# steineggerlab/Metabuli

Hardware: AMD Instinct MI355X
Metric: Mreads/s classified (metabuli classify hot path, reads + index resident in HBM) (higher is better)
Workload: dtype u64

## Files before the change

### metabuli_amd/csrc/kernels_score.h

```cpp
#ifndef MTB_KERNELS_SCORE_H
#define MTB_KERNELS_SCORE_H
#include "dev_util.h"
#include "mtb_core.h"
#include "kernels_join.h"
#include "mtb_score_par.h"

#ifdef MTB_SCORE_PHASE_CYCLES
#define MTB_NPHASE 16
__device__ unsigned long long mtb_phase_cycles[MTB_NPHASE];
__shared__ unsigned long long mtb_phase_lds[MTB_NPHASE];
#define MTB_PHASE_BEGIN() unsigned long long ph_t0_ = __builtin_readcyclecounter()
#define MTB_PHASE_MARK(k) do { unsigned long long t_ = __builtin_readcyclecounter(); if (threadIdx.x == 0) mtb_phase_lds[k] += t_ - ph_t0_; ph_t0_ = t_; } while (0)
#define MTB_PHASE_KERNEL_BEGIN() do { if (threadIdx.x < MTB_NPHASE) mtb_phase_lds[threadIdx.x] = 0; __syncthreads(); } while (0)
#define MTB_PHASE_KERNEL_END() do { __syncthreads(); if (threadIdx.x < MTB_NPHASE) atomicAdd(&mtb_phase_cycles[threadIdx.x], mtb_phase_lds[threadIdx.x]); } while (0)
#else
#define MTB_PHASE_BEGIN() do {} while (0)
#define MTB_PHASE_MARK(k) do {} while (0)
#define MTB_PHASE_KERNEL_BEGIN() do {} while (0)
#define MTB_PHASE_KERNEL_END() do {} while (0)
#endif

#ifndef MTB_SCORE_LDS
#define MTB_SCORE_LDS 160
#endif
// ... 6 lines not shown
    uint64_t b = mtb_sws_bytes<uint32_t>(n);
    b += nb * 12 + (MTB_LR_MAXE + MTB_LR_MAXE * MTB_LR_K) * 4 + ((nb + 15) & ~15ull);
    return (b + 63) & ~63ull;
}

__global__ __launch_bounds__(64) void k_taxcnt_bound(const uint64_t *__restrict__ seg_start, const uint32_t *__restrict__ cursor,
                                                      const int32_t *__restrict__ qlen, const int32_t *__restrict__ qlen2, uint64_t n_reads,
                                                      int32_t dna_shift, uint32_t *__restrict__ bound) {
    uint64_t r = (uint64_t)blockIdx.x * 64 + threadIdx.x;
    if (r >= n_reads) return;
    uint64_t nb = (uint64_t)mtb_num_buckets(qlen[r] + qlen2[r], dna_shift);
    if (cursor) { bound[r] = (uint32_t)nb; return; }
    uint64_t n = seg_start[r + 1] - seg_start[r];
    bound[r] = (uint32_t)(n < nb ? n : nb);
}

__global__ __launch_bounds__(256) void k_count_flags(const uint8_t *__restrict__ f, uint64_t n, unsigned long long *__restrict__ out) {
    uint32_t c = 0;
    for (uint64_t i = (uint64_t)blockIdx.x * 256 + threadIdx.x; i < n; i += (uint64_t)gridDim.x * 256) c += f[i] == 1 ? 1u : 0u;
    for (int d = 32; d > 0; d >>= 1) c += __shfl_down(c, d, 64);
    if ((threadIdx.x & 63) == 0 && c) atomicAdd(out, (unsigned long long)c);
}

__global__ __launch_bounds__(256) void k_list_flag2(const uint8_t *__restrict__ f, uint64_t n, uint32_t *__restrict__ list, uint32_t *__restrict__ n_list) {
    __shared__ uint32_t s_w[4]; __shared__ uint32_t s_base;
    const uint64_t r = (uint64_t)blockIdx.x * 256 + threadIdx.x;
    const bool on = r < n && f[r] == 2;
    const uint64_t m = __ballot(on);
    const uint32_t wv = threadIdx.x >> 6, lane = threadIdx.x & 63u;
    if (lane == 0) s_w[wv] = (uint32_t)__popcll(m);
    __syncthreads();
    if (threadIdx.x == 0) { const uint32_t tot = s_w[0] + s_w[1] + s_w[2] + s_w[3]; s_base = tot ? atomicAdd(n_list, tot) : 0u; }
    __syncthreads();
    if (on) {
        uint32_t at = s_base + (uint32_t)__popcll(m & ((1ull << lane) - 1ull));
        for (uint32_t q = 0; q < wv; q++) at += s_w[q];
        list[at] = (uint32_t)r;
    }
}

__global__ __launch_bounds__(256) void k_list_large(const uint64_t *__restrict__ seg_start, uint64_t n_reads, uint32_t threshold,
                                                     uint32_t *__restrict__ large, uint32_t *__restrict__ n_large, uint32_t *__restrict__ max_seg) {
    uint64_t r = (uint64_t)blockIdx.x * 256 + threadIdx.x;
    uint32_t n = 0;
    if (r < n_reads) {
        n = (uint32_t)(seg_start[r + 1] - seg_start[r]);
        if (n > threshold) large[atomicAdd(n_large, 1u)] = (uint32_t)r;
    }
    for (int d = 32; d > 0; d >>= 1) { uint32_t o = __shfl_down(n, d, 64); n = o > n ? o : n; }
    if ((threadIdx.x & 63) == 0 && n > threshold) atomicMax(max_seg, n);
}

__device__ __forceinline__ int32_t taxcnt_gather_wave(const int32_t *btax, const uint8_t *bham, int32_t nb, int32_t *otax, uint32_t *ocnt, int32_t cap) {
    const int32_t lane = (int32_t)threadIdx.x;
    int32_t ntc = 0;
    int32_t last = -1;
    while (ntc < cap) {
        int32_t mn = INT32_MAX;
        for (int32_t q = lane; q < nb; q += 64) if (bham[q] != 255) { int32_t t = btax[q]; if (t > last && t < mn) mn = t; }
        for (int d = 32; d > 0; d >>= 1) { int32_t o = __shfl_xor(mn, d, 64); mn = o < mn ? o : mn; }
// ... 490 lines not shown
                                               mtb_tax_view tx, mtb_score_params sp, const uint64_t *__restrict__ tc_off,
                                               mtb_result *__restrict__ results, int32_t *__restrict__ tc_tax,
                                               uint32_t *__restrict__ tc_cnt, uint64_t tc_cap, uint8_t *__restrict__ slabs,
                                               uint64_t slab_bytes, uint32_t slab_max_n, uint32_t slab_max_nb,
                                               mtb_match *__restrict__ sorted_out, uint64_t tc_base,
                                               const uint32_t *__restrict__ list, const uint32_t *__restrict__ n_list,
                                               const uint32_t *__restrict__ cursor, uint32_t stride, int seg_by_list,
                                               uint32_t direct, uint32_t epoch, uint32_t *__restrict__ big_list, uint32_t *__restrict__ n_big_out,
                                               uint32_t *__restrict__ cnt_out, unsigned long long *__restrict__ work,
                                               const uint8_t *__restrict__ only_flagged, const uint32_t *__restrict__ seg_cnt = nullptr) {
    __shared__ __attribute__((aligned(16))) uint8_t s_ws[MTB_SCORE_WS_BYTES_(CAP)];
    __shared__ uint32_t s_pf[64];
    static_assert(CAP * sizeof(mtb_path) >= MTB_SCORE_BKT * 13 + (MTB_LR_MAXE + MTB_LR_MAXE * MTB_LR_K) * 4, "decide arrays must fit the path area");
    const uint32_t lane = threadIdx.x;
    MTB_BEGIN_ACQUIRE();
    MTB_PHASE_KERNEL_BEGIN();
    const uint64_t n_iter = list ? (uint64_t)*n_list : n_reads;
    for (uint64_t it = DYN ? (uint64_t)__shfl(lane == 0 ? atomicAdd(work, 1ull) : 0ull, 0, 64) : (uint64_t)blockIdx.x; it < n_iter;
         it = DYN ? (uint64_t)__shfl(lane == 0 ? atomicAdd(work, 1ull) : 0ull, 0, 64) : it + gridDim.x) {
#ifdef MTB_SCORE_PHASE_CYCLES
        unsigned long long kt0_ = __builtin_readcyclecounter();
#endif
        const uint64_t r = list ? (uint64_t)list[it] : it;
        if ((SLOT || DYN) && only_flagged && only_flagged[r] != 1) continue;
        if (SLOT && !DYN && !list && !only_flagged && it + gridDim.x < n_iter) {
            const uint32_t lines = (stride * (uint32_t)sizeof(mtb_slot16) + 127u) / 128u;
            if (lane < lines) {
                const uint8_t *pf = (const uint8_t *)((const mtb_slot16 *)matches + (it + gridDim.x) * (uint64_t)stride) + (uint64_t)lane * 128u;
                __builtin_amdgcn_global_load_lds((const __attribute__((address_space(1))) void *)pf,
                                                 (__attribute__((address_space(3))) void *)s_pf, 4, 0, 0);
            }
        }
        uint64_t s0 = 0; int32_t n = 0;
        if (!SLOT) {
            const uint64_t si = seg_by_list ? it : r;
            s0 = seg_start[si]; n = (DYN && seg_cnt) ? (int32_t)seg_cnt[si] : (int32_t)(seg_start[si + 1] - s0);
        }
        const int32_t ql1 = qlen[r], ql2 = qlen2[r];
        const int32_t read_len = ql1 + ql2;
        mtb_result R = mtb_result_blank(ql1, ql2, 0);
        const int32_t nb = mtb_num_buckets(read_len, sp.dna_shift);
        const uint64_t off = tc_off[r], room = tc_off[r + 1] - off;
        if (SLOT) {
            const uint32_t cur = cursor[r], tail_cap = stride - direct;
            mtb_sws<uint16_t> w;
            mtb_sws_carve<uint16_t>(&w, s_ws, CAP);
            bool defer = cur > tail_cap || nb > MTB_SCORE_BKT;
            if (!defer) {
                uint32_t cnt = 0;
                score_sync<uint16_t>();
#ifdef MTB_SCORE_PHASE_CYCLES
// ... 165 lines not shown
```

### metabuli_amd/csrc/kernels_score_fast.h

```cpp
#ifndef MTB_KERNELS_SCORE_FAST_H
#define MTB_KERNELS_SCORE_FAST_H
#include "dev_util.h"
#include "kernels_score.h"
#include "mtb_core.h"
#include "mtb_score_par.h"

#define MTB_FAST_BKT 128
#ifndef MTB_FAST_MERGE_SINGLES
#define MTB_FAST_MERGE_SINGLES 0
#endif

#ifdef MTB_FAST_DEBUG
__device__ unsigned long long mtb_fast_reasons[32];
#define MTB_FAST_COUNT(k, v) do { if (threadIdx.x == 0) atomicAdd(&mtb_fast_reasons[k], (unsigned long long)(v)); } while (0)
#define MTB_FAST_T0() unsigned long long ft_ = __builtin_readcyclecounter()
#define MTB_FAST_MARK(k) do { const unsigned long long t_ = __builtin_readcyclecounter(); if (threadIdx.x == 0) s_ph[k] += t_ - ft_; ft_ = t_; } while (0)
#else
#define MTB_FAST_COUNT(k, v) do {} while (0)
#define MTB_FAST_T0() do {} while (0)
#define MTB_FAST_MARK(k) do {} while (0)
#endif

#define MTB_DPP_RED(v, OP) do { \
    { const uint32_t o_ = (uint32_t)__builtin_amdgcn_update_dpp((int)(v), (int)(v), 0x111, 0xF, 0xF, false); (v) = OP((v), o_); } \
// ... 28 lines not shown
    __shared__ uint64_t s_aux[NMAX];
    __shared__ uint64_t s_pp[NMAX];
    __shared__ FastPath s_path[64];
    __shared__ uint32_t s_pf[64];
    __shared__ uint32_t s_tl[(BYFRAME || MTB_FAST_MERGE_SINGLES) ? 64 : 1];
    typedef uint32_t __attribute__((may_alias)) u32a; typedef int32_t __attribute__((may_alias)) i32a;
    static_assert(NMAX * 8 >= 2 * MTB_FAST_BKT * 4 && NMAX * 8 >= 256 * 4 && NMAX * 8 >= (MTB_LR_MAXE + MTB_LR_MAXE * MTB_LR_K) * 4, "tables fit the arrays they live in");
    u32a *const s_hcnt = (u32a *)s_pp;
    u32a *const s_hmin = (u32a *)s_key; i32a *const s_btax = (i32a *)s_key + MTB_FAST_BKT;
    i32a *const s_otax = (i32a *)s_pp; u32a *const s_ocnt = (u32a *)s_pp + MTB_FAST_BKT;
    i32a *const s_lev = (i32a *)s_aux; i32a *const s_anc = (i32a *)s_aux + MTB_LR_MAXE;
    const int32_t lane = (int32_t)threadIdx.x;
    MTB_BEGIN_ACQUIRE();
#ifdef MTB_FAST_DEBUG
    __shared__ unsigned long long s_ph[16];
    if (threadIdx.x < 16) s_ph[threadIdx.x] = 0;
#endif
    const uint64_t lt = lanemask_lt();
    const uint64_t le = lt | (1ull << lane);
    const uint32_t tail_cap = stride - direct;
    const uint32_t div_m = (65536u + (uint32_t)sp.dna_shift - 1u) / (uint32_t)sp.dna_shift;
    const uint32_t lines = (stride * (uint32_t)sizeof(mtb_slot16) + 127u) / 128u;

    for (uint64_t r = blockIdx.x; r < n_reads; r += gridDim.x) {
        if (r + gridDim.x < n_reads && (uint32_t)lane < lines) {
            const uint8_t *pf = (const uint8_t *)(slots_all + (r + gridDim.x) * (uint64_t)stride) + (uint64_t)lane * 128u;
            __builtin_amdgcn_global_load_lds((const __attribute__((address_space(1))) void *)pf, (__attribute__((address_space(3))) void *)s_pf, 4, 0, 0);
        }
        MTB_FAST_T0();
        const int32_t ql1 = qlen[r], ql2 = qlen2[r];
        const int32_t read_len = ql1 + ql2;
        const int32_t nb = mtb_num_buckets(read_len, sp.dna_shift);
        const uint32_t cur = cursor[r];
        const mtb_slot16 *slots = slots_all + r * (uint64_t)stride;
        mtb_slot16 x[KL];
#pragma unroll
        for (int k = 0; k < KL; k++) { const uint32_t i = (uint32_t)lane + 64u * k; x[k].a = 0; x[k].b = 0; if (i < stride) x[k] = slots[i]; }
        bool slow = cur > tail_cap || nb > MTB_FAST_BKT;
        wave_fence();
        MTB_FAST_MARK(0);
        int32_t n = 0, n_live = 0;
        uint32_t spc[KL]; bool live[KL]; int32_t dst[KL];
        uint32_t smin = 0xFFFFFFFFu, smax = 0u;
#pragma unroll
        for (int k = 0; k < KL; k++) {
            const uint32_t i = (uint32_t)lane + 64u * k;
            live[k] = i < stride && mtb_slot_epoch(x[k]) == epoch && (i < direct || i - direct < cur);
            spc[k] = live[k] ? (uint32_t)(x[k].a >> 32) : 0xFFFFFFFFu;
            dst[k] = 0;
            n_live += (int32_t)__popcll(__ballot(live[k]));
            smin = spc[k] < smin ? spc[k] : smin;
            if (live[k]) smax = spc[k] > smax ? spc[k] : smax;
        }
        smin = wave_min_u32(smin); smax = wave_max_u32(smax);
        uint32_t todo_min = 0xFFFFFFFFu;
        if (smin != smax) {
            for (int32_t q = lane; q < 256; q += 64) s_hcnt[q] = 0;
            wave_fence();
#pragma unroll
            for (int k = 0; k < KL; k++) if (live[k]) atomicAdd(&s_hcnt[(spc[k] * 0x9E3779B1u) >> 24], 1u);
            wave_fence();
// ... 84 lines not shown
                            if (!same_run(ku, kt)) continue;
                            n_tl_less += (less(ku, kt) || (!less(kt, ku) && u < t)) ? 1u : 0u; n_tl_before += u < t ? 1u : 0u;
                        }
                        const int32_t run_start = ti - (int32_t)n_dir_run - (int32_t)n_tl_before;
#pragma unroll
                        for (int k = 0; k < K; k++) if (lane + 64 * k == ti) np[k] = run_start + (int32_t)(n_dir_less + n_tl_less);
                    }
                    wave_fence();
#pragma unroll
                    for (int k = 0; k < K; k++) { const int32_t i = lane + 64 * k; if (k < nsl && i < n) { s_key[np[k]] = ke[k]; s_aux[np[k]] = ax[k] & ~(1ull << 63); } }
                    wave_fence();
                }
            }
        }
        FKey key[K]; uint32_t tid[K], reh[K];
        int32_t tcanon[K]; uint8_t euk[K];
        const mtb_tax_node *nodes = (const mtb_tax_node *)tx.node;
        bool bhead[K], linked[K];
        int32_t shv[K];
        uint64_t bmask[K + 1], lmask[K + 1], rmask[K];
        const int32_t nslot = (n + 63) >> 6;
        bool bad = false, bad2 = false;
#ifdef MTB_FAST_DEBUG
        if (slow) MTB_FAST_COUNT(cur > tail_cap || nb > MTB_FAST_BKT ? 0 : 1, 1);
#endif
#pragma unroll
        for (int k = 0; k < K; k++) {
            const int32_t i = lane + 64 * k;
            key[k].lo = 0; key[k].hi = 0; tid[k] = 0; reh[k] = 0; bhead[k] = true; linked[k] = false; shv[k] = 0; tcanon[k] = -1; euk[k] = 0;
            bmask[k] = ~0ull; lmask[k] = 0; rmask[k] = 0;
            if (k < nslot && !slow) {
                FKey pk; pk.lo = 0; pk.hi = 0;
                if (i < n) {
                    key[k] = s_key[i]; const uint64_t a = s_aux[i]; tid[k] = (uint32_t)a; reh[k] = (uint32_t)(a >> 32) & 0xFFFFu; if (i > 0) pk = s_key[i - 1];
                }
                {
                    const int32_t t_ = (int32_t)tid[k], s_ = (int32_t)fk_species(key[k]);
                    const bool tv = i < n && t_ >= 0 && t_ <= tx.max_taxid, sv = i < n && s_ >= 0 && s_ <= tx.max_taxid;
                    const int32_t tc_ = nodes[tv ? t_ : 0].canon; const uint8_t eu_ = tx.under_euk[sv ? s_ : 0];
                    tcanon[k] = tv ? tc_ : -1; euk[k] = sv ? eu_ : 0;
                }
                const bool first = i == 0;
                if (i < n && !first) {
                    if (pk.hi > key[k].hi || (pk.hi == key[k].hi && pk.lo > key[k].lo)) bad = true;
                    if (pk.hi == key[k].hi && ((pk.lo ^ key[k].lo) >> 27) == 0) bad2 = true;
                }
                bhead[k] = i >= n || first || ((pk.hi ^ key[k].hi) >> 7) != 0;
                if (i < n && !bhead[k]) {
                    const int32_t pos = (int32_t)fk_pos(key[k]), ppos = (int32_t)fk_pos(pk);
                    const int32_t s = (pos - ppos) / 3;
                    if (s > 0 && s <= sp.max_codon_shift) {
                        shv[k] = s;
                        const bool fwd = fk_frame(key[k]) < 3u;
                        linked[k] = mtb_consecutive(fk_dna(pk), fk_dna(key[k]), s, fwd, sp.kmer_format);
                    }
                }
                bmask[k] = __ballot(bhead[k]);
                lmask[k] = __ballot(linked[k]);
                rmask[k] = __ballot(i < n && !linked[k]);
            }
        }
        bmask[K] = ~0ull; lmask[K] = 0;
#ifdef MTB_FAST_DEBUG
        if (!slow) { if (__any(bad)) MTB_FAST_COUNT(2, 1); else if (__any(bad2)) MTB_FAST_COUNT(3, 1); }
#endif
        slow = slow || __any(bad || bad2);
        if (slow) { if (lane == 0) slow_flag[r] = cur > tail_cap ? 2 : 1; continue; }
        if (lane == 0) cnt_out[r] = (uint32_t)n_live;
        MTB_FAST_MARK(2);
        float ps[K]; int32_t phd[K]; int32_t root[K];
        bool cand[K];
        {
            float carry_s = 0.0f; int32_t carry_hd = 0, last_root = 0;
#pragma unroll
            for (int k = 0; k < K; k++) {
                ps[k] = 0.0f; phd[k] = 0; root[k] = 0; cand[k] = false;
                if (k < nslot) {
                    const int32_t i = lane + 64 * k;
                    float is = 0.0f; int32_t ihd = 0;
                    if (linked[k]) mtb_link_inc(reh[k], shv[k], &is, &ihd);
                    ps[k] = wave_inclusive_scan_dpp(is) + carry_s; phd[k] = wave_inclusive_scan_dpp(ihd) + carry_hd;
                    carry_s = rl_f(ps[k], 63); carry_hd = rl_i(phd[k], 63);
                    const uint64_t mr = rmask[k];
                    const uint64_t lo_roots = mr & le;
                    root[k] = lo_roots ? 64 * k + 63 - (int32_t)__builtin_clzll(lo_roots) : last_root;
                    if (mr) last_root = 64 * k + 63 - (int32_t)__builtin_clzll(mr);
                    if (i < n) s_pp[i] = (uint64_t)__float_as_uint(ps[k]) | ((uint64_t)(uint32_t)phd[k] << 32);
                    const uint64_t bnext = (bmask[k] >> 1) | ((bmask[k + 1] & 1ull) << 63);
                    const uint64_t lnext = (lmask[k] >> 1) | ((lmask[k + 1] & 1ull) << 63);
                    const bool has_next = !((bnext >> lane) & 1ull);
// ... 200 lines not shown
```

### metabuli_amd/csrc/kernels_score_many.h

```cpp
#ifndef MTB_KERNELS_SCORE_MANY_H
#define MTB_KERNELS_SCORE_MANY_H
#include "dev_util.h"
#include "mtb_core.h"
#include "kernels_join.h"
#include "kernels_score.h"
#include "kernels_score_long.h"
#include "kernels_seg_order.h"

#define MTB_MANY_CLAIM 16u
#define MTB_MANY_HASH 1024u

__global__ __launch_bounds__(256) void k_ovf_count(const uint32_t *__restrict__ cursor, const uint8_t *__restrict__ off, uint64_t n_reads, uint32_t tail_cap,
                                                    uint32_t *__restrict__ novf) {
    const uint64_t r = (uint64_t)blockIdx.x * 256 + threadIdx.x;
    if (r >= n_reads) return;
    const uint32_t cur = cursor[r];
    const uint32_t n = (cur > tail_cap && !(off && off[r])) ? cur - tail_cap : 0u;
    novf[r] = n <= 65535u ? n : 0u;
}
__global__ __launch_bounds__(256) void k_ovf_group(const mtb_match *__restrict__ ovf, uint64_t n_ovf, const uint64_t *__restrict__ start, const uint32_t *__restrict__ novf,
                                                    uint32_t *__restrict__ ocur, mtb_match *__restrict__ out, uint64_t region_cap, const unsigned long long *__restrict__ counters) {
    uint64_t i = (uint64_t)blockIdx.x * 256 + threadIdx.x;
    if (region_cap) {
        const unsigned long long cnt = counters[8 * blockIdx.y];
// ... 100 lines not shown
            s_u[j] = ((uint64_t)(uint32_t)m.species_id << 41) | ((uint64_t)mtb_q_frame(m.qinfo) << 38) | ((uint64_t)(mtb_q_pos(m.qinfo) & 0x7FFu) << 27) |
                     ((uint64_t)(m.hamming & 7u) << 24) | (m.dna & 0xFFFFFFu);
        }
        __syncthreads();
        so_bitonic(s_u, s_idx, n, tid);
        mtb_match *dst = big + big_start[b];
        for (uint32_t j = tid; j < n; j += MTB_MSORT_NT) {
            const mtb_match m = fetch(s_idx[j]);
            uint64_t *d = (uint64_t *)(dst + j); const uint64_t *q = (const uint64_t *)&m;
            d[0] = q[0]; d[1] = q[1]; d[2] = q[2];
        }
        if (tid == 0) seg_cnt[b] = n;
    }
}
__global__ __launch_bounds__(256) void k_list_flagged(const uint32_t *__restrict__ list, uint32_t n_list, const uint8_t *__restrict__ todo, const uint32_t *__restrict__ big_cnt,
                                                       uint32_t *__restrict__ rest, uint32_t *__restrict__ n_rest, uint32_t *__restrict__ cnt_out) {
    const uint32_t b = blockIdx.x * 256 + threadIdx.x;
    if (b >= n_list) return;
    const uint32_t r = list[b];
    if (todo[r]) rest[atomicAdd(n_rest, 1u)] = r;
    else cnt_out[r] = big_cnt[b];
}

template <bool KEY64, int CAP>
__global__ __launch_bounds__(64, (CAP > 192 ? 2 : 3)) void k_score_many(const mtb_slot16 *__restrict__ slots_all, uint32_t stride, uint32_t direct, uint32_t epoch,
                                                       const uint32_t *__restrict__ cursor, const uint8_t *__restrict__ off_reads,
                                                       const mtb_match *__restrict__ ovfg, const uint64_t *__restrict__ ovf_start,
                                                       const uint32_t *__restrict__ list, const uint32_t *__restrict__ n_list,
                                                       const int32_t *__restrict__ qlen, const int32_t *__restrict__ qlen2, mtb_tax_view tx, mtb_score_params sp,
                                                       const uint64_t *__restrict__ tc_off, mtb_result *__restrict__ results, int32_t *__restrict__ tc_tax,
                                                       uint32_t *__restrict__ tc_cnt, uint64_t tc_cap, uint64_t tc_base,
                                                       uint32_t *__restrict__ rest_list, uint32_t *__restrict__ n_rest, uint32_t *__restrict__ cnt_out,
                                                       unsigned long long *__restrict__ work, unsigned long long *__restrict__ stats ) {
    __shared__ __attribute__((aligned(16))) uint8_t s_ws[MTB_SCORE_WS_BYTES_(CAP)];
    static_assert(MTB_SCORE_WS_BYTES_(CAP) - CAP * sizeof(mtb_match) >= MTB_MANY_HASH * 8, "the species table fits behind the match records");
    static_assert(CAP * sizeof(mtb_path) >= MTB_SCORE_BKT * 13 + (MTB_LR_MAXE + MTB_LR_MAXE * MTB_LR_K) * 4, "decide arrays must fit the path area");
    uint32_t *const h_key = (uint32_t *)(s_ws + CAP * sizeof(mtb_match));
    uint32_t *const h_val = h_key + MTB_MANY_HASH;
    __shared__ uint32_t s_tfull;
    const uint32_t lane = threadIdx.x;
    const uint64_t lt = lanemask_lt();
    const uint32_t tail_cap = stride - direct;
    MTB_BEGIN_ACQUIRE();
    const uint64_t n_iter = (uint64_t)*n_list;
    unsigned long long seen = 0, kept = 0;
    for (uint64_t c0 = (uint64_t)__shfl(lane == 0 ? atomicAdd(work, (unsigned long long)MTB_MANY_CLAIM) : 0ull, 0, 64); c0 < n_iter;
         c0 = (uint64_t)__shfl(lane == 0 ? atomicAdd(work, (unsigned long long)MTB_MANY_CLAIM) : 0ull, 0, 64))
    for (uint64_t it = c0; it < c0 + MTB_MANY_CLAIM && it < n_iter; it++) {
        const uint64_t r = (uint64_t)list[it];
        const int32_t ql1 = qlen[r], ql2 = qlen2[r];
        const int32_t read_len = ql1 + ql2;
        const int32_t nb = mtb_num_buckets(read_len, sp.dna_shift);
        const uint32_t cur = cursor[r];
        const uint32_t tail_n = cur < tail_cap ? cur : tail_cap;
        uint64_t o0 = 0; uint32_t n_ov = 0;
        if (ovf_start) { o0 = ovf_start[r]; n_ov = (uint32_t)(ovf_start[r + 1] - o0); }
        bool hand_on = (off_reads && off_reads[r]) || nb > MTB_SCORE_BKT || cur - tail_n != n_ov;
        uint32_t why = 2;
        if (!hand_on && cur > 3u * (uint32_t)CAP) { hand_on = true; why = 4; }
        const mtb_slot16 *slots = slots_all + r * (uint64_t)stride;
        mtb_sws<uint16_t> w;
        mtb_sws_carve<uint16_t>(&w, s_ws, CAP);
        uint32_t n = 0, n_all = 0;
        if (!hand_on) {
            score_sync<uint16_t>();
            for (uint32_t q = lane; q < MTB_MANY_HASH; q += 64) { h_key[q] = 0xFFFFFFFFu; h_val[q] = 0u; }
            if (lane == 0) s_tfull = 0;
            score_sync<uint16_t>();
            bool full = false;
            auto enter = [&](uint32_t s, uint32_t f) {
                if (*(volatile uint32_t *)&s_tfull) { full = true; return; }
                uint32_t h = (s * 0x9E3779B1u) >> 22;
                for (uint32_t p = 0; p < MTB_MANY_HASH; p++) {
                    const uint32_t old = atomicCAS(&h_key[h], 0xFFFFFFFFu, s);
                    if (old == 0xFFFFFFFFu || old == s) {
                        const uint32_t bit = 1u << f;
                        if (atomicOr(&h_val[h], bit) & bit) atomicOr(&h_val[h], bit << 8);
                        return;
                    }
                    h = (h + 1u) & (MTB_MANY_HASH - 1u);
                }
                full = true; s_tfull = 1;
            };
            for (uint32_t c0 = 0; c0 < stride; c0 += 64) {
                const uint32_t i = c0 + lane;
                mtb_slot16 x; x.a = 0; x.b = 0;
                if (i < stride) x = slots[i];
                const bool live = i < stride && seg_slot_live(x, i, direct, tail_n, epoch);
                if (live) enter((uint32_t)(x.a >> 32), (uint32_t)(x.b >> 52) & 7u);
                n_all += (uint32_t)__popcll(__ballot(live));
            }
            for (uint32_t c0 = 0; c0 < n_ov; c0 += 64) {
                const uint32_t i = c0 + lane;
                if (i < n_ov) { const mtb_match m = ovfg[o0 + i]; enter((uint32_t)m.species_id, mtb_q_frame(m.qinfo)); }
            }
            n_all += n_ov;
            score_sync<uint16_t>();
            uint32_t used = 0;
            for (uint32_t q = lane; q < MTB_MANY_HASH; q += 64) used += h_key[q] != 0xFFFFFFFFu ? 1u : 0u;
            for (int d = 32; d > 0; d >>= 1) used += (uint32_t)__shfl_xor((int)used, d, 64);
            hand_on = __any(full) || used > MTB_MANY_HASH / 4u * 3u;
            why = 3;
            if (!hand_on) {
                auto alive = [&](uint32_t s) -> bool {
                    uint32_t h = (s * 0x9E3779B1u) >> 22;
                    for (uint32_t p = 0; p < MTB_MANY_HASH; p++) {
                        const uint32_t k = h_key[h];
                        if (k == s) return (h_val[h] >> 8) != 0u;
                        if (k == 0xFFFFFFFFu) return false;
                        h = (h + 1u) & (MTB_MANY_HASH - 1u);
                    }
                    return false;
                };
                uint64_t *dst64 = (uint64_t *)w.m;
                auto put = [&](uint32_t pos, const mtb_match &m) {
                    const uint64_t *q = (const uint64_t *)&m;
                    dst64[3 * pos] = q[0]; dst64[3 * pos + 1] = q[1]; dst64[3 * pos + 2] = q[2];
                };
                for (uint32_t c0 = 0; c0 < stride; c0 += 64) {
                    const uint32_t i = c0 + lane;
                    mtb_slot16 x; x.a = 0; x.b = 0;
                    if (i < stride) x = slots[i];
                    const bool keep = i < stride && seg_slot_live(x, i, direct, tail_n, epoch) && alive((uint32_t)(x.a >> 32));
                    const uint64_t mask = __ballot(keep);
                    const uint32_t pos = n + (uint32_t)__popcll(mask & lt);
                    if (keep && pos < (uint32_t)CAP) put(pos, mtb_slot_unpack(x, (uint32_t)r + 1));
                    n += (uint32_t)__popcll(mask);
                }
                for (uint32_t c0 = 0; c0 < n_ov; c0 += 64) {
                    const uint32_t i = c0 + lane;
                    mtb_match m; m.qinfo = 0; m.target_id = 0; m.species_id = 0; m.dna = 0; m.right_end_hamming = 0; m.hamming = 0; m.pad = 0;
                    bool keep = false;
                    if (i < n_ov) { m = ovfg[o0 + i]; keep = alive((uint32_t)m.species_id); }
                    const uint64_t mask = __ballot(keep);
                    const uint32_t pos = n + (uint32_t)__popcll(mask & lt);
                    if (keep && pos < (uint32_t)CAP) { m.pad = 0; put(pos, m); }
                    n += (uint32_t)__popcll(mask);
                }
                hand_on = n > (uint32_t)CAP;
                why = 4;
                score_sync<uint16_t>();
            }
        }
        if (hand_on) { if (lane == 0) { rest_list[atomicAdd(n_rest, 1u)] = (uint32_t)r; if (stats) atomicAdd(&stats[why], 1ull); } continue; }
        seen += n_all; kept += n;
        mtb_result R = mtb_result_blank(ql1, ql2, 0);
        if (lane == 0) cnt_out[r] = n_all;
        if (n == 0) { if (lane == 0) results[r] = R; continue; }
        const uint64_t off = tc_off[r], room = tc_off[r + 1] - off;
        int32_t *s_btax = (int32_t *)w.path, *s_otax = s_btax + MTB_SCORE_BKT;
        uint32_t *s_ocnt = (uint32_t *)(s_otax + MTB_SCORE_BKT);
        int32_t *s_lev = (int32_t *)(s_ocnt + MTB_SCORE_BKT), *s_anc = s_lev + MTB_LR_MAXE;
        uint8_t *s_bham = (uint8_t *)(s_anc + MTB_LR_MAXE * MTB_LR_K);
        score_read_par<uint16_t, true, KEY64, mtb_match, true, CAP>(w.m, (int32_t)n, w, s_btax, s_bham, s_otax, s_ocnt, s_lev, s_anc, nb, read_len, tx, sp, off, room,
                                                                   tc_tax, tc_cnt, tc_cap, (mtb_match *)nullptr, R);
        if (lane == 0) { R.query_length = ql1; R.query_length2 = ql2; R.reserved = 0; R.taxcnt_off += (uint32_t)tc_base; results[r] = R; }
    }
    if (stats && lane == 0 && seen) { atomicAdd(&stats[0], seen); atomicAdd(&stats[1], kept); }
}

#endif
```

### metabuli_amd/csrc/mtb_api.hip

```cpp
#include <hip/hip_runtime.h>

#include <fcntl.h>
#include <sys/stat.h>
#include <unistd.h>

#include <atomic>
#include <chrono>
#include <condition_variable>
#include <mutex>
#include <functional>
#include <map>
#include <string>
#include <thread>
#include <vector>

#include "../../include/mtb.h"
#include "host_db.h"
#include "host/merge_plan.h"
#include "kernels_extract.h"
#include "kernels_extract_blocks.h"
#include "kernels_index.h"
#include "kernels_join.h"
#include "kernels_build.h"
#include "kernels_merge.h"
// ... 934 lines not shown
        if (dynamic) grid = std::min<uint32_t>(grid, 256u * 14u);
        if (slab_bytes) {
            while ((uint64_t)grid * slab_bytes > (MTB_SLAB_POOL_MAX) && grid > 64) grid /= 2;
            STCHK(ensure(c, "slabs", (size_t)grid * slab_bytes, &d_slabs, BUF_FIXED));
        }
        unsigned long long *d_work = nullptr;
        if (dynamic) { d_work = scal<unsigned long long>(c, SC_SCORE_WORK) + pass; HIPCHK(hipMemsetAsync(d_work, 0, 8, c->stream)); }
#define MTB_LAUNCH_SCORE(SRT, K, CAPV, DYNV, SLOTV) hipLaunchKernelGGL((k_score<SRT, K, mtb_match, CAPV, DYNV, SLOTV>), dim3(grid), dim3(64), 0, c->stream, S->m, S->seg, n_reads, lens.d_ql, \
        lens.d_ql2, tax_view(ix), sp, (const uint64_t *)d_tcoff, out.d_res, out.d_tc_tax, out.d_tc_cnt, out.tc_cap, d_slabs, slab_bytes, slab_n, slab_nb, (mtb_match *)nullptr,  \
        out.tc_base, S->list, S->n_list, S->cursor, S->stride, S->seg_by_list, S->direct, S->epoch, S->big_list, S->n_big, S->cnt_out, d_work, S->only_flagged, S->seg_cnt)
        ScoreSrc S_rest;
        const bool pairs = p->seq_mode == 2;
        if (S->cursor && pass == 0 && key64 && S->stride <= 384u && !c->opt.no_fast_scorer && !(pairs && c->opt.no_fast_pairs)) {
            uint8_t *d_slow;
            STCHK(ensure(c, "slowflag", n_reads, &d_slow));
            HIPCHK(hipMemsetAsync(d_slow, 0, n_reads, c->stream));
            HIPCHK(scal_clear(c, SC_N_GENERIC));
#define MTB_LAUNCH_FAST(...) hipLaunchKernelGGL((k_score_fast<__VA_ARGS__>), dim3(grid), dim3(64), 0, c->stream, (const mtb_slot16 *)S->m, n_reads, lens.d_ql, lens.d_ql2, tax_view(ix), sp, \
            (const uint64_t *)d_tcoff, out.d_res, out.d_tc_tax, out.d_tc_cnt, out.tc_cap, out.tc_base, S->cursor, S->stride, S->direct, S->epoch, d_slow, S->cnt_out)
            { KTimer ktf(c, MTB_K_SCORE_FAST);
              if (pairs) { if (S->stride <= 192) MTB_LAUNCH_FAST(3, 3, true); else if (S->stride <= 256) MTB_LAUNCH_FAST(4, 4, true); else MTB_LAUNCH_FAST(5, 6, true); }
              else if (S->stride <= 128) MTB_LAUNCH_FAST(2); else if (S->stride <= 192) MTB_LAUNCH_FAST(3); else if (S->stride <= 256) MTB_LAUNCH_FAST(4); else MTB_LAUNCH_FAST(5, 6, false); }
#undef MTB_LAUNCH_FAST
            hipLaunchKernelGGL(k_count_flags, dim3(256), dim3(256), 0, c->stream, (const uint8_t *)d_slow, n_reads, scal<unsigned long long>(c, SC_N_GENERIC));
            if (S->big_list && S->n_big) hipLaunchKernelGGL(k_list_flag2, dim3((uint32_t)((n_reads + 255) / 256)), dim3(256), 0, c->stream, (const uint8_t *)d_slow, n_reads, S->big_list, S->n_big);
            c->fast_used = true;
            S_rest = *S; S_rest.only_flagged = d_slow;
            S = &S_rest;
        }
        KTimer kt(c, pass == 0 ? MTB_K_SCORE : MTB_K_SEGSORT);
        if (S->cursor) {
#define MTB_LAUNCH_SLOT(CAPV) do { if (key64) MTB_LAUNCH_SCORE(true, true, CAPV, false, true); else MTB_LAUNCH_SCORE(true, false, CAPV, false, true); } while (0)
            if (S->cap <= 144) MTB_LAUNCH_SLOT(144);
            else if (S->cap <= 160) MTB_LAUNCH_SLOT(160);
            else if (S->cap <= 224) MTB_LAUNCH_SLOT(224);
            else if (S->cap <= 288) MTB_LAUNCH_SLOT(288);
            else MTB_LAUNCH_SLOT(320);
#undef MTB_LAUNCH_SLOT
        } else if (dynamic) {
            if (!S->sort) MTB_LAUNCH_SCORE(false, false, MTB_SCORE_LDS, true, false);
            else if (key64) MTB_LAUNCH_SCORE(true, true, MTB_SCORE_LDS, true, false); else MTB_LAUNCH_SCORE(true, false, MTB_SCORE_LDS, true, false);
        }
        else if (S->sort) { if (key64) MTB_LAUNCH_SCORE(true, true, MTB_SCORE_LDS, false, false); else MTB_LAUNCH_SCORE(true, false, MTB_SCORE_LDS, false, false); }
        else if (S->cap >= 320) MTB_LAUNCH_SCORE(false, false, 320, false, false);
        else MTB_LAUNCH_SCORE(false, false, MTB_SCORE_LDS, false, false);
#undef MTB_LAUNCH_SCORE
    }
    HIPCHK(hipGetLastError());
    return MTB_OK;
}
// ... 1119 lines not shown
        const bool no_many = c->opt.no_score_many != 0;
        uint32_t *d_novf = nullptr; uint64_t *d_ostart = nullptr; mtb_match *d_ovfg = nullptr;
        if (!no_many && sl.stride <= 384u) {
            KTimer ktm(c, MTB_K_SCORE_MANY);
            uint32_t *d_ocur = nullptr, *d_rest;
            STCHK(ensure(c, "restlist", n_reads, &d_rest));
            const bool have_ovf = sl.ovf_region ? c->ovf_max_region != 0 : sl.n_ovf != 0;
            if (have_ovf) {
                STCHK(ensure(c, "novf", n_reads, &d_novf)); STCHK(ensure(c, "ocur", n_reads, &d_ocur)); STCHK(ensure(c, "ovfstart", n_reads + 1, &d_ostart));
                STCHK(scratch(c, "ovfg", sl.n_ovf + 1, &d_ovfg));
                HIPCHK(hipMemsetAsync(d_ocur, 0, n_reads * 4, st));
                hipLaunchKernelGGL(k_ovf_count, dim3((uint32_t)((n_reads + 255) / 256)), dim3(256), 0, st, (const uint32_t *)sl.d_rc, sl.d_off_reads, n_reads, sl.stride - sl.direct, d_novf);
                scan_launch<uint32_t, uint64_t, false>(st, d_novf, n_reads, true, d_ostart, d_ws2);
                if (sl.ovf_region) hipLaunchKernelGGL(k_ovf_group, dim3((uint32_t)((c->ovf_max_region + 255) / 256), MTB_OVF_STRIPES), dim3(256), 0, st, (const mtb_match *)sl.d_ovf, sl.n_ovf,
                                                   (const uint64_t *)d_ostart, (const uint32_t *)d_novf, d_ocur, d_ovfg, sl.ovf_region, (const unsigned long long *)c->d_ovfctr);
                else hipLaunchKernelGGL(k_ovf_group, dim3((uint32_t)((sl.n_ovf + 255) / 256)), dim3(256), 0, st, (const mtb_match *)sl.d_ovf, sl.n_ovf,
                                        (const uint64_t *)d_ostart, (const uint32_t *)d_novf, d_ocur, d_ovfg, (uint64_t)0, (const unsigned long long *)nullptr);
            }
            unsigned long long *d_ms;
            STCHK(ensure(c, "manystat", 16, &d_ms));
            HIPCHK(hipMemsetAsync(d_ms, 0, 16 * 8, st));
            const bool cap192 = c->opt.many_cap ? c->opt.many_cap <= 192 : sl.stride <= 192u;
            const uint32_t gridm = std::min<uint32_t>(n_big, 256u * (cap192 ? 12u : 7u));
#define MTB_LAUNCH_MANY(K64, CAPV) hipLaunchKernelGGL((k_score_many<K64, CAPV>), dim3(gridm), dim3(64), 0, st, (const mtb_slot16 *)sl.d_segm, sl.stride, sl.direct, sl.epoch, (const uint32_t *)sl.d_rc, sl.d_off_reads, \
            (const mtb_match *)d_ovfg, (const uint64_t *)d_ostart, (const uint32_t *)d_biglist, scal<const uint32_t>(c, SC_N_DEFERRED), SL.lens.d_ql, SL.lens.d_ql2, tax_view(ix), SL.sp, SL.d_tcoff, SL.out.d_res, \
            SL.out.d_tc_tax, SL.out.d_tc_cnt, SL.out.tc_cap, SL.out.tc_base, d_rest, (uint32_t *)d_ms, d_cnt, d_ms + 1, d_ms + 2)
            if (cap192) { if (SL.key64) MTB_LAUNCH_MANY(true, 192); else MTB_LAUNCH_MANY(false, 192); }
            else { if (SL.key64) MTB_LAUNCH_MANY(true, 320); else MTB_LAUNCH_MANY(false, 320); }
#undef MTB_LAUNCH_MANY
            HIPCHK(hipGetLastError());
            uint64_t ms4[8] = {0, 0, 0, 0, 0, 0, 0, 0};
            STCHK(d2h(c, ms4, d_ms, 64));
            const uint32_t n_rest = (uint32_t)(ms4[0] & 0xFFFFFFFFull);
            c->many_stats[1] = n_big - n_rest; c->many_stats[2] = ms4[2]; c->many_stats[3] = ms4[3];
            if (c->opt.many_verbose) fprintf(stderr, "mtb: k_score_many: %u reads listed, %u handed on (routed off / buckets / counts %llu, species table full %llu, survivors beyond the staging %llu); %llu matches, %llu survive the dead-species drop\n",
                                                    n_big, n_rest, (unsigned long long)ms4[4], (unsigned long long)ms4[5], (unsigned long long)ms4[6], (unsigned long long)ms4[2], (unsigned long long)ms4[3]);
            n_big = n_rest;
            const unsigned long long *d_nleft = d_ms;
            if (n_big && SL.key64 && !c->opt.no_many_sort) {
                uint32_t *d_bc3, *d_segcnt, *d_rest2; uint64_t *d_bs3; uint8_t *d_todo; mtb_match *d_big3;
                STCHK(ensure(c, "bigcnt", n_big, &d_bc3)); STCHK(ensure(c, "bigstart", (uint64_t)n_big + 1, &d_bs3)); STCHK(ensure(c, "bigseg", n_big, &d_segcnt));
                STCHK(ensure(c, "restlist2", n_reads, &d_rest2)); STCHK(ensure(c, "todoflag", n_reads, &d_todo));
                hipLaunchKernelGGL(k_big_count, dim3(std::min<uint32_t>(n_big, 4096)), dim3(64), 0, st, (const mtb_slot16 *)sl.d_segm, sl.stride, sl.direct, sl.epoch,
                                   (const uint32_t *)sl.d_rc, (const uint32_t *)d_rest, n_big, d_bc3, d_bigidx, scal<uint32_t>(c, SC_MAX_BIG_SEG), sl.d_off_reads);
                scan_launch<uint32_t, uint64_t, false>(st, d_bc3, n_big, true, d_bs3, d_ws2);
                uint64_t total3 = 0;
                STCHK(d2h(c, &total3, d_bs3 + n_big, 8));
                STCHK(scratch(c, "manym", total3 + 1, &d_big3));
                HIPCHK(hipMemsetAsync(d_todo, 0, n_reads, st));
                hipLaunchKernelGGL((k_many_sort<11, 2048u>), dim3(std::min<uint32_t>(n_big, 256u * 8u)), dim3(MTB_MSORT_NT), 0, st, (const mtb_slot16 *)sl.d_segm, sl.stride, sl.direct, sl.epoch, (const uint32_t *)sl.d_rc, sl.d_off_reads,
                                   (const mtb_match *)d_ovfg, (const uint64_t *)d_ostart, (const uint32_t *)d_rest, n_big, SL.lens.d_ql, SL.lens.d_ql2, SL.sp.dna_shift, (const uint64_t *)d_bs3, d_big3, d_segcnt, d_todo, 0u, 2u);
// ... 1670 lines not shown
```

Measured before the change: 71.64.

## Compact slow-read list for rest pass and prefetch next read in score kernels

Replaces the flag-count and flag2 listing kernels with one kernel that builds compact lists of both slow (flag 1) and deferred (flag 2) reads. The rest scoring pass now iterates that list with a grid sized to the slow count, instead of scanning every read and skipping unflagged ones. The fast kernel early-exits reads that are slow by bucket or tail criteria before loading slots, and software-pipelines the qlen/cursor loads for the next read. k_score_many loads slots into registers once (new KL template parameter) instead of reading them twice, and prefetches the next read's slots into LDS. The cost is an extra device-to-host sync to read the slow count, plus more register pressure in k_score_many.

```diff
diff --git a/metabuli_amd/csrc/kernels_score.h b/metabuli_amd/csrc/kernels_score.h
--- a/metabuli_amd/csrc/kernels_score.h
+++ b/metabuli_amd/csrc/kernels_score.h
@@ -52,20 +52,26 @@
     if ((threadIdx.x & 63) == 0 && c) atomicAdd(out, (unsigned long long)c);
 }
 
-__global__ __launch_bounds__(256) void k_list_flag2(const uint8_t *__restrict__ f, uint64_t n, uint32_t *__restrict__ list, uint32_t *__restrict__ n_list) {
-    __shared__ uint32_t s_w[4]; __shared__ uint32_t s_base;
+__global__ __launch_bounds__(256) void k_list_flags(const uint8_t *__restrict__ f, uint64_t n, uint32_t *__restrict__ list1, uint32_t *__restrict__ n_list1,
+                                                     uint32_t *__restrict__ list2, uint32_t *__restrict__ n_list2) {
+    __shared__ uint32_t s_w[2][4]; __shared__ uint32_t s_base[2];
     const uint64_t r = (uint64_t)blockIdx.x * 256 + threadIdx.x;
-    const bool on = r < n && f[r] == 2;
-    const uint64_t m = __ballot(on);
+    const uint8_t fl = r < n ? f[r] : (uint8_t)0;
+    const bool on1 = fl == 1, on2 = fl == 2 && list2;
+    const uint64_t m1 = __ballot(on1), m2 = __ballot(on2);
     const uint32_t wv = threadIdx.x >> 6, lane = threadIdx.x & 63u;
-    if (lane == 0) s_w[wv] = (uint32_t)__popcll(m);
+    if (lane == 0) { s_w[0][wv] = (uint32_t)__popcll(m1); s_w[1][wv] = (uint32_t)__popcll(m2); }
     __syncthreads();
-    if (threadIdx.x == 0) { const uint32_t tot = s_w[0] + s_w[1] + s_w[2] + s_w[3]; s_base = tot ? atomicAdd(n_list, tot) : 0u; }
+    if (threadIdx.x < 2) {
+        const uint32_t tot = s_w[threadIdx.x][0] + s_w[threadIdx.x][1] + s_w[threadIdx.x][2] + s_w[threadIdx.x][3];
+        s_base[threadIdx.x] = tot ? atomicAdd(threadIdx.x ? n_list2 : n_list1, tot) : 0u;
+    }
     __syncthreads();
-    if (on) {
-        uint32_t at = s_base + (uint32_t)__popcll(m & ((1ull << lane) - 1ull));
-        for (uint32_t q = 0; q < wv; q++) at += s_w[q];
-        list[at] = (uint32_t)r;
+    if (on1 || on2) {
+        const int w = on2 ? 1 : 0;
+        uint32_t at = s_base[w] + (uint32_t)__popcll((on2 ? m2 : m1) & ((1ull << lane) - 1ull));
+        for (uint32_t q = 0; q < wv; q++) at += s_w[w][q];
+        (on2 ? list2 : list1)[at] = (uint32_t)r;
     }
 }
 
@@ -602,11 +608,13 @@
         unsigned long long kt0_ = __builtin_readcyclecounter();
 #endif
         const uint64_t r = list ? (uint64_t)list[it] : it;
+        const bool pf_next = SLOT && !DYN && !only_flagged && it + gridDim.x < n_iter;
+        const uint64_t r_next = !pf_next ? 0 : list ? (uint64_t)list[it + gridDim.x] : it + gridDim.x;
         if ((SLOT || DYN) && only_flagged && only_flagged[r] != 1) continue;
-        if (SLOT && !DYN && !list && !only_flagged && it + gridDim.x < n_iter) {
+        if (pf_next) {
             const uint32_t lines = (stride * (uint32_t)sizeof(mtb_slot16) + 127u) / 128u;
             if (lane < lines) {
-                const uint8_t *pf = (const uint8_t *)((const mtb_slot16 *)matches + (it + gridDim.x) * (uint64_t)stride) + (uint64_t)lane * 128u;
+                const uint8_t *pf = (const uint8_t *)((const mtb_slot16 *)matches + r_next * (uint64_t)stride) + (uint64_t)lane * 128u;
                 __builtin_amdgcn_global_load_lds((const __attribute__((address_space(1))) void *)pf,
                                                  (__attribute__((address_space(3))) void *)s_pf, 4, 0, 0);
             }
diff --git a/metabuli_amd/csrc/kernels_score_fast.h b/metabuli_amd/csrc/kernels_score_fast.h
--- a/metabuli_amd/csrc/kernels_score_fast.h
+++ b/metabuli_amd/csrc/kernels_score_fast.h
@@ -74,21 +74,25 @@
     const uint32_t div_m = (65536u + (uint32_t)sp.dna_shift - 1u) / (uint32_t)sp.dna_shift;
     const uint32_t lines = (stride * (uint32_t)sizeof(mtb_slot16) + 127u) / 128u;
 
+    int32_t ql1_nx = 0, ql2_nx = 0; uint32_t cur_nx = 0;
+    if (blockIdx.x < n_reads) { ql1_nx = qlen[blockIdx.x]; ql2_nx = qlen2[blockIdx.x]; cur_nx = cursor[blockIdx.x]; }
     for (uint64_t r = blockIdx.x; r < n_reads; r += gridDim.x) {
         if (r + gridDim.x < n_reads && (uint32_t)lane < lines) {
             const uint8_t *pf = (const uint8_t *)(slots_all + (r + gridDim.x) * (uint64_t)stride) + (uint64_t)lane * 128u;
             __builtin_amdgcn_global_load_lds((const __attribute__((address_space(1))) void *)pf, (__attribute__((address_space(3))) void *)s_pf, 4, 0, 0);
         }
         MTB_FAST_T0();
-        const int32_t ql1 = qlen[r], ql2 = qlen2[r];
+        const int32_t ql1 = ql1_nx, ql2 = ql2_nx;
         const int32_t read_len = ql1 + ql2;
         const int32_t nb = mtb_num_buckets(read_len, sp.dna_shift);
-        const uint32_t cur = cursor[r];
+        const uint32_t cur = cur_nx;
+        if (r + gridDim.x < n_reads) { ql1_nx = qlen[r + gridDim.x]; ql2_nx = qlen2[r + gridDim.x]; cur_nx = cursor[r + gridDim.x]; }
+        if (cur > tail_cap || nb > MTB_FAST_BKT) { MTB_FAST_COUNT(0, 1); if (lane == 0) slow_flag[r] = cur > tail_cap ? 2 : 1; continue; }
         const mtb_slot16 *slots = slots_all + r * (uint64_t)stride;
         mtb_slot16 x[KL];
 #pragma unroll
         for (int k = 0; k < KL; k++) { const uint32_t i = (uint32_t)lane + 64u * k; x[k].a = 0; x[k].b = 0; if (i < stride) x[k] = slots[i]; }
-        bool slow = cur > tail_cap || nb > MTB_FAST_BKT;
+        bool slow = false;
         wave_fence();
         MTB_FAST_MARK(0);
         int32_t n = 0, n_live = 0;
@@ -219,7 +223,7 @@
         const int32_t nslot = (n + 63) >> 6;
         bool bad = false, bad2 = false;
 #ifdef MTB_FAST_DEBUG
-        if (slow) MTB_FAST_COUNT(cur > tail_cap || nb > MTB_FAST_BKT ? 0 : 1, 1);
+        if (slow) MTB_FAST_COUNT(1, 1);
 #endif
 #pragma unroll
         for (int k = 0; k < K; k++) {
@@ -262,7 +266,7 @@
         if (!slow) { if (__any(bad)) MTB_FAST_COUNT(2, 1); else if (__any(bad2)) MTB_FAST_COUNT(3, 1); }
 #endif
         slow = slow || __any(bad || bad2);
-        if (slow) { if (lane == 0) slow_flag[r] = cur > tail_cap ? 2 : 1; continue; }
+        if (slow) { if (lane == 0) slow_flag[r] = 1; continue; }
         if (lane == 0) cnt_out[r] = (uint32_t)n_live;
         MTB_FAST_MARK(2);
         float ps[K]; int32_t phd[K]; int32_t root[K];
diff --git a/metabuli_amd/csrc/kernels_score_many.h b/metabuli_amd/csrc/kernels_score_many.h
--- a/metabuli_amd/csrc/kernels_score_many.h
+++ b/metabuli_amd/csrc/kernels_score_many.h
@@ -146,7 +146,7 @@
     else cnt_out[r] = big_cnt[b];
 }
 
-template <bool KEY64, int CAP>
+template <bool KEY64, int CAP, int KL>
 __global__ __launch_bounds__(64, (CAP > 192 ? 2 : 3)) void k_score_many(const mtb_slot16 *__restrict__ slots_all, uint32_t stride, uint32_t direct, uint32_t epoch,
                                                        const uint32_t *__restrict__ cursor, const uint8_t *__restrict__ off_reads,
                                                        const mtb_match *__restrict__ ovfg, const uint64_t *__restrict__ ovf_start,
@@ -162,9 +162,11 @@
     uint32_t *const h_key = (uint32_t *)(s_ws + CAP * sizeof(mtb_match));
     uint32_t *const h_val = h_key + MTB_MANY_HASH;
     __shared__ uint32_t s_tfull;
+    __shared__ uint32_t s_pf[64];
     const uint32_t lane = threadIdx.x;
     const uint64_t lt = lanemask_lt();
     const uint32_t tail_cap = stride - direct;
+    const uint32_t lines = (stride * (uint32_t)sizeof(mtb_slot16) + 127u) / 128u;
     MTB_BEGIN_ACQUIRE();
     const uint64_t n_iter = (uint64_t)*n_list;
     unsigned long long seen = 0, kept = 0;
@@ -172,6 +174,8 @@
          c0 = (uint64_t)__shfl(lane == 0 ? atomicAdd(work, (unsigned long long)MTB_MANY_CLAIM) : 0ull, 0, 64))
     for (uint64_t it = c0; it < c0 + MTB_MANY_CLAIM && it < n_iter; it++) {
         const uint64_t r = (uint64_t)list[it];
+        const bool have_next = it + 1 < c0 + MTB_MANY_CLAIM && it + 1 < n_iter;
+        const uint64_t r_next = have_next ? (uint64_t)list[it + 1] : 0;
         const int32_t ql1 = qlen[r], ql2 = qlen2[r];
         const int32_t read_len = ql1 + ql2;
         const int32_t nb = mtb_num_buckets(read_len, sp.dna_shift);
@@ -187,6 +191,15 @@
         mtb_sws_carve<uint16_t>(&w, s_ws, CAP);
         uint32_t n = 0, n_all = 0;
         if (!hand_on) {
+            mtb_slot16 x[KL];
+            mtb_match m0; m0.qinfo = 0; m0.target_id = 0; m0.species_id = 0; m0.dna = 0; m0.right_end_hamming = 0; m0.hamming = 0; m0.pad = 0;
+#pragma unroll
+            for (int k = 0; k < KL; k++) { const uint32_t i = lane + 64u * k; x[k].a = 0; x[k].b = 0; if (i < stride) x[k] = slots[i]; }
+            if (lane < n_ov) m0 = ovfg[o0 + lane];
+            if (have_next && lane < lines) {
+                const uint8_t *pf = (const uint8_t *)(slots_all + r_next * (uint64_t)stride) + (uint64_t)lane * 128u;
+                __builtin_amdgcn_global_load_lds((const __attribute__((address_space(1))) void *)pf, (__attribute__((address_space(3))) void *)s_pf, 4, 0, 0);
+            }
             score_sync<uint16_t>();
             for (uint32_t q = lane; q < MTB_MANY_HASH; q += 64) { h_key[q] = 0xFFFFFFFFu; h_val[q] = 0u; }
             if (lane == 0) s_tfull = 0;
@@ -206,16 +219,17 @@
                 }
                 full = true; s_tfull = 1;
             };
-            for (uint32_t c0 = 0; c0 < stride; c0 += 64) {
-                const uint32_t i = c0 + lane;
-                mtb_slot16 x; x.a = 0; x.b = 0;
-                if (i < stride) x = slots[i];
-                const bool live = i < stride && seg_slot_live(x, i, direct, tail_n, epoch);
-                if (live) enter((uint32_t)(x.a >> 32), (uint32_t)(x.b >> 52) & 7u);
-                n_all += (uint32_t)__popcll(__ballot(live));
-            }
-            for (uint32_t c0 = 0; c0 < n_ov; c0 += 64) {
-                const uint32_t i = c0 + lane;
+            bool live[KL];
+#pragma unroll
+            for (int k = 0; k < KL; k++) {
+                const uint32_t i = lane + 64u * k;
+                live[k] = i < stride && seg_slot_live(x[k], i, direct, tail_n, epoch);
+                if (live[k]) enter((uint32_t)(x[k].a >> 32), (uint32_t)(x[k].b >> 52) & 7u);
+                n_all += (uint32_t)__popcll(__ballot(live[k]));
+            }
+            if (lane < n_ov) enter((uint32_t)m0.species_id, mtb_q_frame(m0.qinfo));
+            for (uint32_t c1 = 64; c1 < n_ov; c1 += 64) {
+                const uint32_t i = c1 + lane;
                 if (i < n_ov) { const mtb_match m = ovfg[o0 + i]; enter((uint32_t)m.species_id, mtb_q_frame(m.qinfo)); }
             }
             n_all += n_ov;
@@ -241,21 +255,19 @@
                     const uint64_t *q = (const uint64_t *)&m;
                     dst64[3 * pos] = q[0]; dst64[3 * pos + 1] = q[1]; dst64[3 * pos + 2] = q[2];
                 };
-                for (uint32_t c0 = 0; c0 < stride; c0 += 64) {
-                    const uint32_t i = c0 + lane;
-                    mtb_slot16 x; x.a = 0; x.b = 0;
-                    if (i < stride) x = slots[i];
-                    const bool keep = i < stride && seg_slot_live(x, i, direct, tail_n, epoch) && alive((uint32_t)(x.a >> 32));
+#pragma unroll
+                for (int k = 0; k < KL; k++) {
+                    const bool keep = live[k] && alive((uint32_t)(x[k].a >> 32));
                     const uint64_t mask = __ballot(keep);
                     const uint32_t pos = n + (uint32_t)__popcll(mask & lt);
-                    if (keep && pos < (uint32_t)CAP) put(pos, mtb_slot_unpack(x, (uint32_t)r + 1));
+                    if (keep && pos < (uint32_t)CAP) put(pos, mtb_slot_unpack(x[k], (uint32_t)r + 1));
                     n += (uint32_t)__popcll(mask);
                 }
-                for (uint32_t c0 = 0; c0 < n_ov; c0 += 64) {
-                    const uint32_t i = c0 + lane;
-                    mtb_match m; m.qinfo = 0; m.target_id = 0; m.species_id = 0; m.dna = 0; m.right_end_hamming = 0; m.hamming = 0; m.pad = 0;
+                for (uint32_t c1 = 0; c1 < n_ov; c1 += 64) {
+                    const uint32_t i = c1 + lane;
+                    mtb_match m = m0;
                     bool keep = false;
-                    if (i < n_ov) { m = ovfg[o0 + i]; keep = alive((uint32_t)m.species_id); }
+                    if (i < n_ov) { if (c1) m = ovfg[o0 + i]; keep = alive((uint32_t)m.species_id); }
                     const uint64_t mask = __ballot(keep);
                     const uint32_t pos = n + (uint32_t)__popcll(mask & lt);
                     if (keep && pos < (uint32_t)CAP) { m.pad = 0; put(pos, m); }
@@ -265,6 +277,9 @@
                 why = 4;
                 score_sync<uint16_t>();
             }
+        } else if (have_next && lane < lines) {
+            const uint8_t *pf = (const uint8_t *)(slots_all + r_next * (uint64_t)stride) + (uint64_t)lane * 128u;
+            __builtin_amdgcn_global_load_lds((const __attribute__((address_space(1))) void *)pf, (__attribute__((address_space(3))) void *)s_pf, 4, 0, 0);
         }
         if (hand_on) { if (lane == 0) { rest_list[atomicAdd(n_rest, 1u)] = (uint32_t)r; if (stats) atomicAdd(&stats[why], 1ull); } continue; }
         seen += n_all; kept += n;
diff --git a/metabuli_amd/csrc/mtb_api.hip b/metabuli_amd/csrc/mtb_api.hip
--- a/metabuli_amd/csrc/mtb_api.hip
+++ b/metabuli_amd/csrc/mtb_api.hip
@@ -980,10 +980,17 @@
               if (pairs) { if (S->stride <= 192) MTB_LAUNCH_FAST(3, 3, true); else if (S->stride <= 256) MTB_LAUNCH_FAST(4, 4, true); else MTB_LAUNCH_FAST(5, 6, true); }
               else if (S->stride <= 128) MTB_LAUNCH_FAST(2); else if (S->stride <= 192) MTB_LAUNCH_FAST(3); else if (S->stride <= 256) MTB_LAUNCH_FAST(4); else MTB_LAUNCH_FAST(5, 6, false); }
 #undef MTB_LAUNCH_FAST
-            hipLaunchKernelGGL(k_count_flags, dim3(256), dim3(256), 0, c->stream, (const uint8_t *)d_slow, n_reads, scal<unsigned long long>(c, SC_N_GENERIC));
-            if (S->big_list && S->n_big) hipLaunchKernelGGL(k_list_flag2, dim3((uint32_t)((n_reads + 255) / 256)), dim3(256), 0, c->stream, (const uint8_t *)d_slow, n_reads, S->big_list, S->n_big);
+            uint32_t *d_slowlist;
+            STCHK(ensure(c, "slowlist", n_reads, &d_slowlist));
+            const bool defer_list = S->big_list && S->n_big;
+            hipLaunchKernelGGL(k_list_flags, dim3((uint32_t)((n_reads + 255) / 256)), dim3(256), 0, c->stream, (const uint8_t *)d_slow, n_reads, d_slowlist, scal<uint32_t>(c, SC_N_GENERIC),
+                               defer_list ? S->big_list : (uint32_t *)nullptr, defer_list ? S->n_big : (uint32_t *)nullptr);
             c->fast_used = true;
-            S_rest = *S; S_rest.only_flagged = d_slow;
+            uint64_t n_slow = 0;
+            STCHK(d2h(c, &n_slow, scal<uint64_t>(c, SC_N_GENERIC), 8));
+            n_slow &= 0xFFFFFFFFull;
+            S_rest = *S; S_rest.list = d_slowlist; S_rest.n_list = scal<const uint32_t>(c, SC_N_GENERIC);
+            grid = (uint32_t)std::max<uint64_t>(1, std::min<uint64_t>(n_slow, std::max<uint64_t>(256ull * 14, n_slow / 8)));
             S = &S_rest;
         }
         KTimer kt(c, pass == 0 ? MTB_K_SCORE : MTB_K_SEGSORT);
@@ -2149,11 +2156,12 @@
             HIPCHK(hipMemsetAsync(d_ms, 0, 16 * 8, st));
             const bool cap192 = c->opt.many_cap ? c->opt.many_cap <= 192 : sl.stride <= 192u;
             const uint32_t gridm = std::min<uint32_t>(n_big, 256u * (cap192 ? 12u : 7u));
-#define MTB_LAUNCH_MANY(K64, CAPV) hipLaunchKernelGGL((k_score_many<K64, CAPV>), dim3(gridm), dim3(64), 0, st, (const mtb_slot16 *)sl.d_segm, sl.stride, sl.direct, sl.epoch, (const uint32_t *)sl.d_rc, sl.d_off_reads, \
+#define MTB_LAUNCH_MANY(K64, CAPV, KLV) hipLaunchKernelGGL((k_score_many<K64, CAPV, KLV>), dim3(gridm), dim3(64), 0, st, (const mtb_slot16 *)sl.d_segm, sl.stride, sl.direct, sl.epoch, (const uint32_t *)sl.d_rc, sl.d_off_reads, \
             (const mtb_match *)d_ovfg, (const uint64_t *)d_ostart, (const uint32_t *)d_biglist, scal<const uint32_t>(c, SC_N_DEFERRED), SL.lens.d_ql, SL.lens.d_ql2, tax_view(ix), SL.sp, SL.d_tcoff, SL.out.d_res, \
             SL.out.d_tc_tax, SL.out.d_tc_cnt, SL.out.tc_cap, SL.out.tc_base, d_rest, (uint32_t *)d_ms, d_cnt, d_ms + 1, d_ms + 2)
-            if (cap192) { if (SL.key64) MTB_LAUNCH_MANY(true, 192); else MTB_LAUNCH_MANY(false, 192); }
-            else { if (SL.key64) MTB_LAUNCH_MANY(true, 320); else MTB_LAUNCH_MANY(false, 320); }
+            if (cap192 && sl.stride <= 192u) { if (SL.key64) MTB_LAUNCH_MANY(true, 192, 3); else MTB_LAUNCH_MANY(false, 192, 3); }
+            else if (cap192) { if (SL.key64) MTB_LAUNCH_MANY(true, 192, 6); else MTB_LAUNCH_MANY(false, 192, 6); }
+            else { if (SL.key64) MTB_LAUNCH_MANY(true, 320, 6); else MTB_LAUNCH_MANY(false, 320, 6); }
 #undef MTB_LAUNCH_MANY
             HIPCHK(hipGetLastError());
             uint64_t ms4[8] = {0, 0, 0, 0, 0, 0, 0, 0};
```

Measured after the change: 70.89. 1.0% lower.
